# alshai/Big-BWT

Measured on AMD Instinct MI355X. Metric: input MB/s to .bwt (bit-exact vs ref), higher is better.
Workload: dtype u8; 1 GPU; BASELINE configs[2]: 64x mutated yeast-shaped FASTA (~0.79 GB), -w 10 -p 100, BWT + -s -e sampled SA; bytes_per_gpu=787308470, w=10, p=100, flags=6, phrases=16409159, words=921010, dict_bytes=79900101, parallelism=1 GPU

## Files before the change

### big-bwt_amd/csrc/merge.hip

```cpp
#include "kernels.hpp"
#include "prims.hpp"
#include "devutil.hpp"
#include <algorithm>
#include <cstdlib>

namespace pfp {

static constexpr int TB = 256;
constexpr int kOffTileLog = 11;


template <class I> struct alignas(16) Idx8 { I v[8]; };
template <class I>
__global__ __launch_bounds__(256) void slot_payload_kernel(uint64_t N, const I *__restrict__ sa,
                                                           const uint64_t *__restrict__ skeys,
                                                           const uint8_t *__restrict__ refined, const uint8_t *__restrict__ b,
                                                           WordView wv,
                                                           const uint32_t *__restrict__ wocc, uint32_t d, int w,
                                                           uint32_t *__restrict__ cnt, uint8_t *__restrict__ pc) {
  if ((uint64_t)BID * 2048 >= N) return;
  uint64_t t0 = ((uint64_t)BID * 256 + threadIdx.x) * 8;
  uint32_t c8[8], p8[8];
  const int nk = t0 >= N ? 0 : ((N - t0) >= 8 ? 8 : (int)(N - t0));
  uint64_t rf = 0;
// ... 110 lines not shown
  for (int q = 0; q < wv; q++) run += ws[q];
  uint32_t o8[8];
#pragma unroll
  for (int k = 0; k < 8; k++) { o8[k] = (uint32_t)run; run += r8[k].x; }
  *reinterpret_cast<uint4 *>(loc + t0) = make_uint4(o8[0], o8[1], o8[2], o8[3]);
  *reinterpret_cast<uint4 *>(loc + t0 + 4) = make_uint4(o8[4], o8[5], o8[6], o8[7]);
  if (threadIdx.x == 255) {
    tsum[BID] = run;
    if (run >> 32) atomicOr(overflow, 1u);
  }
  if (nk == 8) {
    *reinterpret_cast<uint2 *>(pc + t0) = make_uint2(p8[0] | (p8[1] << 8) | (p8[2] << 16) | (p8[3] << 24),
                                                     p8[4] | (p8[5] << 8) | (p8[6] << 16) | (p8[7] << 24));
    if (sfirst) {
      *reinterpret_cast<uint4 *>(sfirst + t0) = make_uint4(r8[0].y, r8[1].y, r8[2].y, r8[3].y);
      *reinterpret_cast<uint4 *>(sfirst + t0 + 4) = make_uint4(r8[4].y, r8[5].y, r8[6].y, r8[7].y);
    }
    if (slast) {
      *reinterpret_cast<uint4 *>(slast + t0) = make_uint4(r8[0].z, r8[1].z, r8[2].z, r8[3].z);
      *reinterpret_cast<uint4 *>(slast + t0 + 4) = make_uint4(r8[4].z, r8[5].z, r8[6].z, r8[7].z);
    }
    if (ssl) {
      *reinterpret_cast<uint4 *>(ssl + t0) = make_uint4(r8[0].w >> 8, r8[1].w >> 8, r8[2].w >> 8, r8[3].w >> 8);
      *reinterpret_cast<uint4 *>(ssl + t0 + 4) = make_uint4(r8[4].w >> 8, r8[5].w >> 8, r8[6].w >> 8, r8[7].w >> 8);
    }
  } else {
    for (int k = 0; k < nk; k++) {
      pc[t0 + k] = (uint8_t)p8[k];
      if (sfirst) sfirst[t0 + k] = r8[k].y;
      if (slast) slast[t0 + k] = r8[k].z;
      if (ssl) ssl[t0 + k] = r8[k].w >> 8;
    }
  }
#pragma unroll
  for (int k = 0; k < 8; k++) {
    if (k < nk && p8[k] != 0 && g8[k] == prev_g && (any_multi_is_hard || p8[k] != prev_pc)) hard[g8[k]] = 1;
    prev_pc = p8[k]; prev_g = g8[k];
  }
}

template <class I>
__global__ void group_flags_kernel(uint64_t N, const I *__restrict__ grp, const uint8_t *__restrict__ pc,
                                   int any_multi_is_hard, uint8_t *__restrict__ hard) {
  uint64_t t = (uint64_t)BID * blockDim.x + threadIdx.x;
  if (t >= N || pc[t] == 0) return;
  I g = grp[t];
  if (g == t) return;
  if (any_multi_is_hard || pc[t] != pc[g]) hard[g] = 1;
}

enum : uint8_t { CLS_NONE = 0, CLS_FILL = 1, CLS_FULL = 2, CLS_HARD = 3 };
enum : int { SA_NONE = 0, SA_DENSE = 1, SA_SPARSE = 2 };

template <class I>
__global__ void gather_idx_kernel(uint64_t n, const I *__restrict__ idx, const I *__restrict__ src, I *__restrict__ dst) {
  uint64_t i = (uint64_t)BID * blockDim.x + threadIdx.x;
  if (i < n) dst[i] = src[idx[i]];
}
struct alignas(32) WordRec { uint32_t ist, occ, first, last; uint64_t wend, pad; };
__global__ void wistart_kernel(uint32_t d, const uint32_t *__restrict__ lexrank, const uint32_t *__restrict__ istart_lex,
                               const uint32_t *__restrict__ wocc, const uint32_t *__restrict__ ilist,
                               const uint64_t *__restrict__ wend, uint32_t *__restrict__ wistart, WordRec *__restrict__ wrec) {
  uint32_t j = BID * blockDim.x + threadIdx.x;
  if (j >= d) return;
  const uint32_t st = istart_lex[lexrank[j]] + 1;
  wistart[j] = st;
  if (wrec) { const uint32_t oc = wocc[j]; wrec[j] = WordRec{st, oc, ilist[st], ilist[st + oc - 1], wend[j], 0}; }
}

template <class I>
struct MergeArgsT {
  uint64_t N, n_out; uint32_t d; int w; int want_sa;
  uint64_t pos_base, n_out_global;
  uint64_t out_lo, out_hi;
  const I *sa, *grp;
  WordView wv;
  const uint32_t *ist, *wistart;
  const WordRec *wrec;
  const uint32_t *sfirst, *slast, *ssl;
  const uint8_t *pc, *hard, *gmaj;
  const uint64_t *tbase; const uint32_t *loc;
  const uint32_t *ilist; const uint8_t *bwlast; const uint64_t *bwsai;
  const uint32_t *istart_lex, *iword; const uint64_t *wslot_lex; uint64_t slot_base;
  uint8_t *bwt; uint64_t *out_sa;
  int pass;
  const uint64_t *bmap, *bpre;
  uint64_t *sa_c;
};
enum : int { PASS_BWT = 1, PASS_SA = 2 };
template <class I>
__device__ __forceinline__ void sa_put(const MergeArgsT<I> &a, uint64_t x, uint64_t v) {
  if (x < a.out_lo || x >= a.out_hi) return;
  if (!a.bmap) { a.out_sa[x] = v; return; }
  const uint64_t r = x - a.out_lo, wv = a.bmap[r >> 6];
  if (!((wv >> (r & 63)) & 1ull)) return;
  if (a.sa_c) a.sa_c[a.bpre[r >> 6] + (uint64_t)__popcll(wv & ((1ull << (r & 63)) - 1ull))] = v;
  else a.out_sa[x] = v;
}
template <class I>
__device__ __forceinline__ bool sa_wanted(const MergeArgsT<I> &a, uint64_t x) {
  if (x < a.out_lo || x >= a.out_hi) return false;
  if (!a.bmap) return true;
  const uint64_t r = x - a.out_lo;
  return (a.bmap[r >> 6] >> (r & 63)) & 1ull;
}
template <class I>
__device__ __forceinline__ uint64_t slot_off(const MergeArgsT<I> &a, uint64_t t) { return a.tbase[t >> kOffTileLog] + a.loc[t]; }


__device__ __forceinline__ uint8_t fix_char(uint8_t ch) { return ch == kDollar ? 0 : ch; }
template <class I>
__device__ __forceinline__ uint32_t slot_ist(const MergeArgsT<I> &a, uint64_t t) {
  return a.ist ? a.ist[t] : a.wistart[word_of(a.wv, a.sa[t])];
}

template <class I>
__device__ __forceinline__ uint32_t slot_first(const MergeArgsT<I> &a, uint64_t t) { return a.sfirst ? a.sfirst[t] : a.wrec[word_of(a.wv, a.sa[t])].first; }
template <class I>
__device__ __forceinline__ uint32_t slot_last(const MergeArgsT<I> &a, uint64_t t) { return a.slast ? a.slast[t] : a.wrec[word_of(a.wv, a.sa[t])].last; }
template <class I>
__device__ __forceinline__ uint64_t slot_slen(const MergeArgsT<I> &a, uint64_t t) {
  if (a.ssl) { const uint32_t v = a.ssl[t]; if (v != kSlCap) return v; }
  return slen_of(a.wv, a.sa[t]);
}

constexpr int kHardLds = 1024;
constexpr int kHardRank = 512;
constexpr int kHardMem = 256;
constexpr int kHardSortMin = 512;
constexpr int kSlots = 2048;
constexpr uint64_t kExpandQuota = 1u << 16;

template <bool kDense>
struct ExpandLds {
  uint32_t loff[kSlots + 1];
  uint8_t lch[kSlots];
  uint8_t lcls[kDense ? kSlots : 1];
  uint32_t lfist[kDense ? kSlots : 1];
};

template <class I, bool kDense>
__device__ __forceinline__ void expand_stage(const MergeArgsT<I> &a, ExpandLds<kDense> &L, uint64_t t0, int ns, uint64_t base) {
  for (int s = threadIdx.x; s <= ns; s += 256) L.loff[s] = (uint32_t)(slot_off(a, t0 + s) - base);
  for (int s = threadIdx.x; s < ns; s += 256) {
    const uint64_t t = t0 + s;
    const uint8_t pc = a.pc[t];
    uint8_t cls = pc == 0 ? CLS_NONE : (pc == kEndOfWord ? CLS_FULL : CLS_FILL);
    uint8_t ch = 0;
    if (cls == CLS_FILL) {
      ch = fix_char(pc);
      const I g = a.grp[t];
      if (a.hard[g]) {
// ... 83 lines not shown
    for (uint64_t x0 = kExpandQuota + ((uint64_t)BID * 256 + threadIdx.x) * 16; x0 < Ltot; x0 += (uint64_t)GDIM * 256 * 16)
      expand_16(a, L, ns, base, x0, Ltot);
    if constexpr (kDense)
      for (uint64_t x = kExpandQuota + (uint64_t)BID * 256 + threadIdx.x; x < Ltot; x += (uint64_t)GDIM * 256)
        expand_sa_1(a, L, t0, ns, base, x);
  }
}

template <class I>
__device__ __forceinline__ bool word_entry(const MergeArgsT<I> &a, uint64_t e, uint64_t &t, uint64_t &x) {
  const uint32_t q = a.iword[e + 1] - 1u;
  const uint64_t gs = a.wslot_lex[q];
  if (gs < a.slot_base || gs - a.slot_base >= a.N) return false;
  t = gs - a.slot_base;
  x = slot_off(a, t) + (e - (uint64_t)a.istart_lex[q]);
  return true;
}
template <class I>
__global__ __launch_bounds__(256) void word_chars_kernel(MergeArgsT<I> a, uint64_t P) {
  const uint64_t e = (uint64_t)BID * 256 + threadIdx.x;
  if (e >= P) return;
  uint64_t t, x;
  if (!word_entry(a, e, t, x) || x < a.out_lo || x >= a.out_hi) return;
  a.bwt[x] = a.bwlast[a.ilist[e + 1]];
}
template <class I>
__global__ __launch_bounds__(256) void word_sa_kernel(MergeArgsT<I> a, uint64_t P) {
  const uint64_t e = (uint64_t)BID * 256 + threadIdx.x;
  if (e >= P) return;
  uint64_t t, x;
  if (!word_entry(a, e, t, x) || !sa_wanted(a, x)) return;
  const uint64_t pos = a.ilist[e + 1];
  sa_put(a, x, a.pos_base + x == 0 ? a.n_out_global - 1 : a.bwsai[pos] - slot_slen(a, t));
}
__global__ void iword_kernel(uint64_t P, uint32_t d, const uint32_t *__restrict__ istart_lex, uint32_t *__restrict__ iword) {
  const uint64_t e = (uint64_t)BID * blockDim.x + threadIdx.x;
  if (e > P) return;
  if (e == P) { iword[0] = 0; return; }
  uint32_t lo = 0, hi = d;
  while (hi - lo > 1) { const uint32_t mid = (lo + hi) >> 1; if ((uint64_t)istart_lex[mid] <= e) lo = mid; else hi = mid; }
  iword[e + 1] = lo + 1;
}

__device__ __forceinline__ uint32_t lane_read(uint32_t v, int l) { return (uint32_t)__builtin_amdgcn_readlane((int)v, l); }
__device__ __forceinline__ uint64_t lane_read(uint64_t v, int l) {
  return (uint64_t)lane_read((uint32_t)v, l) | ((uint64_t)lane_read((uint32_t)(v >> 32), l) << 32);
}
template <class I>
__global__ __launch_bounds__(256) void unit_edges_kernel(MergeArgsT<I> a) {
  const uint64_t t = (uint64_t)BID * 256 + threadIdx.x;
  const int lane = threadIdx.x & 63;
  const uint64_t wbase = t - lane;
  const bool in = t < a.N;
  const uint32_t ch = in ? a.pc[t] : 0u;
  const bool unit = ch != 0 && ch != kEndOfWord;
  I g = 0;
  if (unit) g = a.grp[t];
  const unsigned long long um = __ballot(unit);
  const I g_next = __shfl_down(g, 1, 64);
  const bool unit_next = (um >> ((lane + 1) & 63)) & 1ull;
  bool cont;
  if (lane < 63) cont = unit && unit_next && g_next == g;
  else cont = unit && t + 1 < a.N && a.pc[t + 1] != 0 && a.pc[t + 1] != kEndOfWord && a.grp[t + 1] == g;
  const unsigned long long cm = __ballot(cont);
  const bool head = unit && (uint64_t)g == t;
  const bool last = unit && !cont;
  uint64_t o_first = 0, o_last = 0;
  if (head) o_first = slot_off(a, t);
  if (last) o_last = slot_off(a, t + 1) - 1;
  const bool need_first = head && sa_wanted(a, o_first);
  const bool need_last = last && sa_wanted(a, o_last);
  const bool head_here = unit && (uint64_t)g >= wbase;
  const int hl = head_here ? (int)((uint64_t)g - wbase) : lane;
  const unsigned long long lm = __ballot(last) >> lane;
  const int ll = lm ? lane + (__ffsll((long long)lm) - 1) : lane;
  const bool nf = head_here && ((__ballot(need_first) >> hl) & 1ull);
  const bool nlz = unit && lm != 0 && ((__ballot(need_last) >> ll) & 1ull);
  uint32_t mn = 0xFFFFFFFFu, mx = 0;
  uint64_t mysl = 0;
  if (nf || nlz) {
    if (nf) mn = slot_first(a, t);
    if (nlz) mx = slot_last(a, t);
    if (need_first || need_last) mysl = slot_slen(a, t);
  }
  const bool do_min = __ballot(nf) != 0, do_max = __ballot(nlz) != 0;
  unsigned long long r = cm & ~(1ull << 63);
#pragma unroll
  for (int o = 1; o < 64; o <<= 1) {
    if (!r) break;
    if (do_min) {
      const uint32_t v = __shfl_down(mn, o, 64);
      if (((r >> lane) & 1ull) && v < mn) mn = v;
    }
    if (do_max) {
      const uint32_t v = __shfl_up(mx, o, 64);
      if (lane >= o && ((r >> (lane - o)) & 1ull) && v > mx) mx = v;
    }
    r &= r >> o;
  }
  const I g63 = lane_read(g, 63);
  const bool cont63 = (cm >> 63) & 1ull;
  const unsigned long long fwd = __ballot(need_first && cont63 && g63 == g);
  if (fwd) {
    uint32_t ext = 0xFFFFFFFFu;
    for (uint64_t m0 = wbase + 64;; m0 += 64) {
      const uint64_t m = m0 + lane;
      const bool mine = m < a.N && a.grp[m] == g63;
      uint32_t f = 0xFFFFFFFFu;
      if (mine) f = slot_first(a, m);
      f = wave_min(f);
      ext = f < ext ? f : ext;
      if (__ballot(mine) != ~0ull) break;
    }
    if ((fwd >> lane) & 1ull) mn = ext < mn ? ext : mn;
  }
  const uint64_t g0 = lane_read(g, 0);
  const unsigned long long bwd = __ballot(need_last && (uint64_t)g < wbase);
  if (bwd && (um & 1ull)) {
    uint32_t ext = 0;
    for (uint64_t m0 = g0; m0 < wbase; m0 += 64) {
      const uint64_t m = m0 + lane;
      uint32_t l = 0;
      if (m < wbase) l = slot_last(a, m);
      l = wave_max(l);
      ext = l > ext ? l : ext;
    }
    if ((bwd >> lane) & 1ull) mx = ext > mx ? ext : mx;
  }
  if (need_first) sa_put(a, o_first, a.bwsai[mn] - mysl);
  if (need_last) sa_put(a, o_last, a.bwsai[mx] - mysl);
}

__device__ __forceinline__ uint32_t pack_byte_flags(uint32_t m) {
  return (m & 1u) | ((m >> 7) & 2u) | ((m >> 14) & 4u) | ((m >> 21) & 8u);
}
__global__ __launch_bounds__(256) void run_bitmap_kernel(const uint8_t *__restrict__ bwt, uint64_t cnt, uint64_t *__restrict__ bmap,
                                                         uint32_t *__restrict__ wcnt, uint64_t *__restrict__ smap,
                                                         uint32_t *__restrict__ scnt, uint64_t *__restrict__ emap,
                                                         uint32_t *__restrict__ ecnt) {
  const uint64_t ch = (uint64_t)BID * 256 + threadIdx.x;
  const uint64_t base = ch * 16;
  uint32_t ms[4], me[4];
  run_mask16(bwt, base, cnt, -1, -1, 0, ms);
  run_mask16(bwt, base, cnt, -1, -1, 1, me);
  uint32_t bs = 0, be = 0;
#pragma unroll
  for (int q = 0; q < 4; q++) { bs |= pack_byte_flags(ms[q]) << (4 * q); be |= pack_byte_flags(me[q]) << (4 * q); }
  uint64_t vs = (uint64_t)bs << (16 * (threadIdx.x & 3)), ve = (uint64_t)be << (16 * (threadIdx.x & 3));
  vs |= __shfl_xor(vs, 1, 64); vs |= __shfl_xor(vs, 2, 64);
  ve |= __shfl_xor(ve, 1, 64); ve |= __shfl_xor(ve, 2, 64);
  if ((threadIdx.x & 3) == 0 && base < cnt) {
    const uint64_t w = ch >> 2;
    bmap[w] = vs | ve; wcnt[w] = (uint32_t)__popcll(vs | ve);
    if (smap) { smap[w] = vs; scnt[w] = (uint32_t)__popcll(vs); }
    if (emap) { emap[w] = ve; ecnt[w] = (uint32_t)__popcll(ve); }
  }
}
__global__ void count_unset_kernel(const uint64_t *__restrict__ v, uint64_t n, unsigned long long *__restrict__ total) {
  const uint64_t i = (uint64_t)BID * blockDim.x + threadIdx.x;
  if (i < n && v[i] == ~0ull) atomicAdd(total, 1ull);
}
struct HardGroupInfo { uint64_t g; uint64_t E; uint32_t k; uint32_t minor; };
struct MinorMember { uint64_t g; uint32_t k, m; uint64_t roff; uint64_t base; uint32_t ist, occ; uint32_t sl; uint32_t ch; };
struct MinorRec { uint64_t o; uint32_t pos, pred, succ, flags, sl, pad; };
template <class I>
__global__ __launch_bounds__(256) void hard_classify_kernel(MergeArgsT<I> a, const I *__restrict__ heads, uint64_t nH,
                                                            uint8_t *__restrict__ gmaj, HardGroupInfo *__restrict__ info,
                                                            uint32_t *__restrict__ minor_cnt, uint8_t *__restrict__ fallback,
                                                            unsigned long long *__restrict__ chars_total, uint32_t *__restrict__ minor_members) {
  const uint64_t h = (uint64_t)BID * 256 + threadIdx.x;
  unsigned long long mychars = 0, myk = 0;
  if (h < nH) {
  const uint64_t g = heads[h];
  uint64_t lo = 1, hi = 2;
  while (g + hi < a.N && a.grp[g + hi] == (I)g) { lo = hi; hi *= 2; }
  if (g + hi > a.N) hi = a.N - g;
  while (hi - lo > 1) { const uint64_t mid = (lo + hi) >> 1; if (a.grp[g + mid] == (I)g) lo = mid; else hi = mid; }
  const uint64_t k = hi;
  const uint64_t base = slot_off(a, g);
  const uint64_t E = slot_off(a, g + k) - base;
  uint32_t c0 = 0x100, c1 = 0x100, c2 = 0x100, c3 = 0x100;
  uint64_t n0 = 0, n1 = 0, n2 = 0, n3 = 0;
  bool many = false;
// ... 99 lines not shown
          bool hp = false, hs = false;
          if (m == me) {
            lb = j;
            if (a.want_sa) {
              if (j > 0) { pv = a.ilist[my_ist + j - 1]; hp = true; }
              if (j + 1 < my_occ) { sv = a.ilist[my_ist + j + 1]; hs = true; }
            }
          } else {
            const uint32_t mfirst = slot_first(a, g + m), mlast = slot_last(a, g + m);
            if (pos < mfirst) { lb = 0; sv = mfirst; hs = true; }
            else if (pos > mlast) { lb = (uint32_t)(slot_off(a, g + m + 1) - slot_off(a, g + m)); pv = mlast; hp = true; }
            else {
              const WordRec wr = a.wrec[word_of(a.wv, a.sa[g + m])];
              const uint32_t *lst = a.ilist + wr.ist;
              uint32_t l2 = 1, h2 = wr.occ - 1;
              while (l2 < h2) { const uint32_t mid = (l2 + h2) >> 1; if (lst[mid] < pos) l2 = mid + 1; else h2 = mid; }
              lb = l2;
              if (a.want_sa) { pv = lst[lb - 1]; hp = true; sv = lst[lb]; hs = true; }
            }
          }
          r += lb;
          if (hp && (!has_pred || pv > pred)) { pred = pv; has_pred = 1; }
          if (hs && (!has_succ || sv < succ)) { succ = sv; has_succ = 1; }
        }
      }
#pragma unroll
      for (int o = 1; o < LPM; o <<= 1) {
        r += __shfl_xor(r, o, 64);
        const uint32_t op = __shfl_xor(pred, o, 64), ohp = __shfl_xor(has_pred, o, 64);
        const uint32_t os = __shfl_xor(succ, o, 64), ohs = __shfl_xor(has_succ, o, 64);
        if (ohp && (!has_pred || op > pred)) { pred = op; has_pred = 1; }
        if (ohs && (!has_succ || os < succ)) { succ = os; has_succ = 1; }
      }
      if (!act || ll != 0) continue;
      const uint64_t o = base + r;
      if (o >= a.out_lo && o < a.out_hi) a.bwt[o] = mych;
      if (a.want_sa)
        recs[mmv.roff + j] = MinorRec{o, pos, pred, succ, has_pred | (has_succ << 1), (uint32_t)sl, 0u};
    }
  }
}

template <class I>
__global__ void hard_minor_sa_kernel(MergeArgsT<I> a, const MinorRec *__restrict__ recs, uint64_t n) {
  const uint64_t q = (uint64_t)BID * blockDim.x + threadIdx.x;
  if (q >= n) return;
  const MinorRec r = recs[q];
  sa_put(a, r.o, a.bwsai[r.pos] - (uint64_t)r.sl);
  if ((r.flags & 1u) && r.o >= 1) sa_put(a, r.o - 1, a.bwsai[r.pred] - (uint64_t)r.sl);
  if (r.flags & 2u) sa_put(a, r.o + 1, a.bwsai[r.succ] - (uint64_t)r.sl);
}

struct BigGroup { uint64_t g; uint64_t E; uint32_t k; uint32_t pad; };
struct HardLds {
  uint32_t lpos[kHardRank];
  uint8_t lq[kHardRank];
  uint32_t lmoff[kHardMem + 1], lmist[kHardMem], lmsl[kHardMem];
  uint8_t lmch[kHardMem], lmg[kHardMem];
  uint64_t gbase[64], ghead[64];
  uint32_t geoff[65], gk0[65];
};
__device__ __forceinline__ void wave_lds_sync() {
  __builtin_amdgcn_wave_barrier();
  __threadfence_block();
}
__device__ __forceinline__ uint32_t wave_max_u32(uint32_t v) {
#pragma unroll
  for (int o = 32; o > 0; o >>= 1) { const uint32_t x = __shfl_xor(v, o, 64); v = x > v ? x : v; }
  return v;
}
template <class I>
__global__ __launch_bounds__(256) void hard_groups_kernel(MergeArgsT<I> a, const I *__restrict__ heads,
                                                          const uint64_t *__restrict__ nheads_p,
                                                          unsigned long long *__restrict__ stats,
                                                          BigGroup *__restrict__ big, uint32_t big_cap,
                                                          BigGroup *__restrict__ mid, uint32_t mid_cap, int gpb) {
  __shared__ HardLds S[4];
  const int wv = threadIdx.x >> 6, lane = threadIdx.x & 63;
  HardLds &L = S[wv];
  const uint64_t nH = *nheads_p;
  const uint64_t nbatch = (nH + gpb - 1) / gpb;
  unsigned long long my_chars = 0, my_groups = 0;
  for (uint64_t b = BID * 4 + wv; b < nbatch; b += GDIM * 4) {
    const uint64_t hidx = b * gpb + lane;
    uint64_t g = 0, base = 0;
    uint32_t k = 0, E = 0;
    bool live = false;
    if (lane < gpb && hidx < nH) {
      g = heads[hidx];
      uint32_t kk = 0;
      while (g + kk < a.N && a.grp[g + kk] == (I)g && a.pc[g + kk] != 0) kk++;
      base = slot_off(a, g);
      const uint64_t Eg = slot_off(a, g + kk) - base;
      if (kk && !(base + Eg <= a.out_lo || base >= a.out_hi)) {
        my_chars += Eg; my_groups += 1;
        const bool sorted_path = Eg > (uint64_t)kHardSortMin;
        if (Eg <= (uint64_t)kHardRank && kk <= (uint32_t)kHardMem && !sorted_path) { live = true; k = kk; E = (uint32_t)Eg; }
        else if (Eg <= (uint64_t)kHardLds && sorted_path) {
          const unsigned long long idx = atomicAdd(&stats[3], 1ull);
          if (idx < mid_cap) mid[idx] = BigGroup{g, Eg, kk, 0};
        } else {
          const unsigned long long idx = atomicAdd(&stats[2], 1ull);
          if (idx < big_cap) big[idx] = BigGroup{g, Eg, kk, 0};
        }
      }
    }
    unsigned long long todo = __ballot(live);
    while (todo) {
      const bool mine = (todo >> lane) & 1ull;
      uint32_t pk = mine ? k : 0u, pE = mine ? E : 0u;
#pragma unroll
      for (int o = 1; o < 64; o <<= 1) {
        const uint32_t vk = __shfl_up(pk, o, 64), vE = __shfl_up(pE, o, 64);
        if (lane >= o) { pk += vk; pE += vE; }
      }
      const bool fit = mine && pk <= (uint32_t)kHardMem && pE <= (uint32_t)kHardRank;
      const unsigned long long take = __ballot(fit);
      todo &= ~take;
      const int nG = __popcll(take);
      const int lastl = 63 - __clzll((long long)take);
      const uint32_t M = __shfl(pk, lastl, 64), Eb = __shfl(pE, lastl, 64);
      if (fit) {
        const int gi = __popcll(take & ((1ull << lane) - 1ull));
        L.ghead[gi] = g; L.gbase[gi] = base; L.geoff[gi] = pE - E; L.gk0[gi] = pk - k;
      }
      if (lane == 0) { L.geoff[nG] = Eb; L.gk0[nG] = M; }
      wave_lds_sync();
      for (uint32_t q = lane; q < M; q += 64) {
        int lo = 0, hi = nG;
        while (hi - lo > 1) { const int mid = (lo + hi) >> 1; if (L.gk0[mid] <= q) lo = mid; else hi = mid; }
        const uint64_t t = L.ghead[lo] + (q - L.gk0[lo]);
        L.lmoff[q] = L.geoff[lo] + (uint32_t)(slot_off(a, t) - L.gbase[lo]);
        L.lmist[q] = slot_ist(a, t);
        uint32_t sl = 0;
        if (a.want_sa) sl = (uint32_t)slot_slen(a, t);
        L.lmsl[q] = sl;
        L.lmch[q] = fix_char(a.pc[t]);
        L.lmg[q] = (uint8_t)lo;
      }
      if (lane == 0) L.lmoff[M] = Eb;
      wave_lds_sync();
      for (uint32_t e = lane; e < Eb; e += 64) {
        uint32_t lo = 0, hi = M;
        while (hi - lo > 1) { const uint32_t mid = (lo + hi) >> 1; if (L.lmoff[mid] <= e) lo = mid; else hi = mid; }
        L.lpos[e] = a.ilist[L.lmist[lo] + (e - L.lmoff[lo])];
        L.lq[e] = (uint8_t)lo;
// ... 156 lines not shown
  }
  uint64_t own = 0;
  for (int k = 0; k < 8; k++) own += v[k];
  uint64_t inc = own;
  const int lane = threadIdx.x & 63, wv = threadIdx.x >> 6;
  for (int o = 1; o < 64; o <<= 1) { const uint64_t u = __shfl_up(inc, o, 64); if (lane >= o) inc += u; }
  if (lane == 63) ws[wv] = inc;
  __syncthreads();
  uint64_t run = inc - own;
  for (int q = 0; q < wv; q++) run += ws[q];
  uint32_t o8[8];
  for (int k = 0; k < 8; k++) { o8[k] = (uint32_t)run; run += v[k]; }
  *reinterpret_cast<uint4 *>(loc + t0) = make_uint4(o8[0], o8[1], o8[2], o8[3]);
  *reinterpret_cast<uint4 *>(loc + t0 + 4) = make_uint4(o8[4], o8[5], o8[6], o8[7]);
  if (threadIdx.x == 255) {
    tsum[BID] = run;
    if (run >> 32) atomicOr(overflow, 1u);
  }
}


enum class RecordSource {
  SortKeys,
  Gathered,
  PerSlot,
};

struct MergeSwitches {
  int prec_direct = -1;
  uint32_t big_cap = 0;
  uint64_t big_budget = 1ull << 27;
  static MergeSwitches read() {
    MergeSwitches s;
    if (const char *e = getenv("PFP_PREC_DIRECT")) s.prec_direct = atoi(e) != 0;
    if (const char *e = getenv("PFP_BIG_CAP")) { if (atoll(e) > 0) s.big_cap = (uint32_t)atoll(e); }
    if (const char *e = getenv("PFP_BIG_BUDGET")) s.big_budget = strtoull(e, nullptr, 10);
    return s;
  }
};

template <class I>
static RecordSource choose_record_source(pfp_ctx *c, uint64_t N, uint64_t NP, int sa_mode, const SuffixOrderT<I> &so, const MergeSwitches &sw) {
  if (sa_mode != SA_DENSE && so.paybits == 16 && so.skeys.p && so.n_refined * 5 < N) return RecordSource::SortKeys;
  bool direct = N * 4 <= NP;
  const uint64_t dev_bytes = c->pool.soft_limit ? c->pool.soft_limit / 7 * 10 : (64ull << 30);
  if (NP * sizeof(PosRec) > dev_bytes / 8) direct = true;
  if (sw.prec_direct >= 0) direct = sw.prec_direct != 0;
  return direct ? RecordSource::PerSlot : RecordSource::Gathered;
}

template <class I>
struct HeadList {
  const I *heads;
  const uint64_t *n_dev;
  uint64_t n;
};

template <class I>
struct Merge {
  pfp_ctx *const c;
  const Dictionary &D;
  const DictIndex &ix;
  const SuffixOrderT<I> &so;
  const ParseBWT &pb;
  const uint32_t *const occ_lex;
  const MergeOpts o;
  BwtOutputs &out;
  const uint64_t NP, N;
  const uint32_t d;
  const int sa_mode;
  const MergeSwitches sw;
  const RecordSource src;
  const WordView wv;
  const uint64_t ntile;
  const uint32_t nblk;
  const int first_pass;

  MergeArgsT<I> a{};
  uint64_t n_out = 0;

  struct {
    DBuf<uint32_t> istart_lex, wistart;
    DBuf<uint32_t> iword;
    DBuf<WordRec> wrec;
  } word;
  struct {
    DBuf<uint8_t> pc, hard;
    DBuf<uint32_t> loc, ovf;
    DBuf<uint64_t> tsum, tbase;
    DBuf<uint32_t> sfirst, slast, ssl;
  } slot;
  enum { kAllHeads = 0, kFallbackHeads = 1 };
  struct {
    DBuf<unsigned long long> hstats;
    uint64_t n_heads = 0;
    uint32_t big_cap = 0, mid_cap = 0;
    DBuf<BigGroup> big, mid;
    DBuf<I> heads;
    DBuf<uint64_t> list_len;
    DBuf<unsigned long long> mstat;
    DBuf<uint8_t> gmaj, fallback;
    DBuf<HardGroupInfo> ginfo;
    DBuf<uint32_t> minor_cnt, mm_cnt;
    DBuf<uint64_t> minor_off, mm_off;
    DBuf<MinorMember> mm_list;
    uint64_t n_mm = 0, sum_k = 0, n_minor = 0;
    DBuf<I> fb_heads;
    DBuf<MinorRec> recs;
    int gpb = 64;
    uint32_t nmid = 0, nbig = 0;
    DBuf<uint64_t> estart;
    std::vector<uint64_t> es;
  } hg;
  DBuf<uint32_t> heavy, nheavy;

  Merge(pfp_ctx *c_, const Dictionary &D_, const DictIndex &ix_, const SuffixOrderT<I> &so_, const ParseBWT &pb_, const uint32_t *occ_lex_,
        const MergeOpts &o_, BwtOutputs &out_)
      : c(c_), D(D_), ix(ix_), so(so_), pb(pb_), occ_lex(occ_lex_), o(o_), out(out_), NP(D_.dsize), N(so_.N), d((uint32_t)D_.d),
        sa_mode(!o_.flags ? SA_NONE : ((o_.flags & PFP_FLAG_SA) ? SA_DENSE : SA_SPARSE)), sw(MergeSwitches::read()),
        src(choose_record_source<I>(c_, N, NP, sa_mode, so_, sw)), wv(word_view(D_, ix_)), ntile((N >> kOffTileLog) + 1),
        nblk((uint32_t)cdiv64(N, kSlots)), first_pass(sa_mode == SA_SPARSE ? PASS_BWT : (PASS_BWT | PASS_SA)) {}

  MergeArgsT<I> with_pass(int pass) const { MergeArgsT<I> x = a; x.pass = pass; return x; }

  void word_records() {
    word.istart_lex.alloc(c, d); word.wistart.alloc(c, d);
    exclusive_sum_u32(c, occ_lex, word.istart_lex.p, d);
    word.wrec.alloc(c, d);
    hipLaunchKernelGGL(wistart_kernel, gdim(cdiv(d, TB)), gdim(TB), 0, c->stream, d, ix.lexrank.p, word.istart_lex.p, D.wocc.p, pb.ilist.p,
                       ix.wend.p, word.wistart.p, word.wrec.p);
    if (!pb.iword.p) {
      word.iword.alloc(c, pb.P + 1);
      hipLaunchKernelGGL(iword_kernel, gdim(cdiv(pb.P + 1, TB)), gdim(TB), 0, c->stream, pb.P, d, word.istart_lex.p, word.iword.p);
    }
  }

  void alloc_slot_tables() {
    slot.pc.alloc(c, N + 8); slot.hard.alloc(c, N);
    slot.loc.alloc(c, ntile << kOffTileLog); slot.ovf.alloc(c, 1);
    alloc_counts(c, slot.tsum, ntile); slot.tbase.alloc(c, ntile + 1);
    slot.hard.zero();
    slot.ovf.zero();
  }
  void slot_tables_from_keys(DBuf<uint32_t> &cnt) {
    { KScope ks(c, "pfp::slot_payload_kernel", N * (8 + 1 + 5));
      hipLaunchKernelGGL(slot_payload_kernel<I>, gdim(cdiv(cdiv64(N, 8), 256)), gdim(256), 0, c->stream, N, so.sa.p, so.skeys.p,
                         so.refined.p, D.bytes.p, wv, D.wocc.p, d, o.w, cnt.p, slot.pc.p); }
    { KScope ks(c, "pfp::slot_loc_kernel", N * 8);
      hipLaunchKernelGGL(slot_loc_kernel, gdim((unsigned)ntile), gdim(256), 0, c->stream, cnt.p, N, slot.loc.p, slot.tsum.p, slot.ovf.p); }
    { KScope ks(c, "pfp::group_flags_kernel", N * 5);
      hipLaunchKernelGGL(group_flags_kernel<I>, gdim(cdiv(N, TB)), gdim(TB), 0, c->stream, N, so.grp.p, slot.pc.p, 0, slot.hard.p); }
  }
  void slot_tables_gathered() {
    const int dense = sa_mode == SA_DENSE ? 1 : 0;
    const uint64_t np256 = cdiv64(NP, 256) * 256;
    DBuf<PosRec> prec(c, np256);
    { KScope ks(c, "pfp::pprec16_kernel", NP * (1 + 16) + (uint64_t)d * 40);
      hipLaunchKernelGGL(pprec16_kernel, gdim(cdiv(np256, TB)), gdim(TB), 0, c->stream, wv, o.w, reinterpret_cast<const uint4 *>(word.wrec.p),
                         dense, (uint64_t)0, NP, prec.p); }
    slot_records(prec.p);
// ... 21 lines not shown

  void fill_args() {
    const bool dense = sa_mode == SA_DENSE;
    a.N = N; a.n_out = n_out; a.d = d; a.w = o.w; a.want_sa = sa_mode;
    a.pos_base = o.pos_base; a.n_out_global = o.n_out_global ? o.n_out_global : n_out;
    a.sa = so.sa.p; a.grp = so.grp.p; a.wv = wv;
    a.ist = dense ? slot.sfirst.p : nullptr;
    a.wistart = word.wistart.p; a.wrec = word.wrec.p;
    a.sfirst = dense ? nullptr : slot.sfirst.p; a.slast = slot.slast.p; a.ssl = slot.ssl.p;
    a.pc = slot.pc.p; a.hard = slot.hard.p; a.tbase = slot.tbase.p; a.loc = slot.loc.p;
    a.ilist = pb.ilist.p; a.bwlast = pb.bwlast.p; a.bwsai = pb.bwsai.p;
    a.istart_lex = word.istart_lex.p; a.iword = pb.iword.p ? pb.iword.p : word.iword.p;
    a.wslot_lex = ix.wslot_lex.p; a.slot_base = so.slot_base;
    a.out_lo = o.out_lo; a.out_hi = o.out_hi < n_out ? o.out_hi : n_out;
    a.bwt = out.d_bwt - o.out_lo; a.out_sa = out.d_sa ? out.d_sa - o.out_lo : nullptr;
  }

  void find_hard_groups() {
    hg.hstats.alloc(c, 5);
    hg.hstats.zero();
    hg.n_heads = count_flags(c, slot.hard.p, N);
    hg.big_cap = sw.big_cap ? sw.big_cap : (uint32_t)std::min<uint64_t>({(uint64_t)1u << 20, hg.n_heads + 1, n_out / 1024 + 1});
    hg.big.alloc(c, hg.big_cap);
    hg.mid_cap = (uint32_t)std::min<uint64_t>(n_out / (kHardSortMin + 1) + 64, 0x7FFFFFFFull);
    hg.mid.alloc(c, hg.mid_cap);
    hg.heads.alloc(c, hg.n_heads + 1);
    hg.list_len.alloc(c, 2);
    select_index<I>(c, slot.hard.p, hg.heads.p, hg.list_len.p + kAllHeads, N);
    hg.mstat.alloc(c, 2);
    hg.mstat.zero();
  }

  HeadList<I> classify() {
    const uint64_t n_heads = hg.n_heads;
    hg.gmaj.alloc(c, N); hg.fallback.alloc(c, n_heads); hg.ginfo.alloc(c, n_heads);
    alloc_counts(c, hg.minor_cnt, n_heads); hg.minor_off.alloc(c, n_heads + 1);
    alloc_counts(c, hg.mm_cnt, n_heads); hg.mm_off.alloc(c, n_heads + 1);
    a.gmaj = hg.gmaj.p;
    { KScope ks(c, "pfp::hard_classify_kernel", n_heads * 40);
      hipLaunchKernelGGL(hard_classify_kernel<I>, gdim(cdiv(n_heads, 256)), gdim(256), 0, c->stream, a, hg.heads.p, n_heads, hg.gmaj.p,
                         hg.ginfo.p, hg.minor_cnt.p, hg.fallback.p, hg.mstat.p, hg.mm_cnt.p); }
    exclusive_sum_u32_u64(c, hg.minor_cnt.p, hg.minor_off.p, n_heads + 1);
    exclusive_sum_u32_u64(c, hg.mm_cnt.p, hg.mm_off.p, n_heads + 1);
    hg.n_mm = read_scalar(c, hg.mm_off.p + n_heads);
    hg.sum_k = read_scalar(c, (const uint64_t *)hg.mstat.p + 1);
    if (hg.n_mm) {
      hg.mm_list.alloc(c, hg.n_mm);
      KScope ks(c, "pfp::hard_minor_fill_kernel", n_heads * 40 + hg.n_mm * 16);
      hipLaunchKernelGGL(hard_minor_fill_kernel<I>, gdim(cdiv(n_heads * 8, 256)), gdim(256), 0, c->stream, a, hg.ginfo.p, n_heads, hg.mm_off.p,
                         hg.minor_off.p, hg.gmaj.p, hg.mm_list.p);
    }
    const uint64_t n_fallback = count_flags(c, hg.fallback.p, n_heads);
    hg.n_minor = read_scalar(c, hg.minor_off.p + n_heads);
    hg.fb_heads.alloc(c, n_fallback + 1);
    {
      DBuf<I> fidx(c, n_fallback + 1);
      select_index<I>(c, hg.fallback.p, fidx.p, hg.list_len.p + kFallbackHeads, n_heads);
      if (n_fallback) hipLaunchKernelGGL(gather_idx_kernel<I>, gdim(cdiv(n_fallback, 256)), gdim(256), 0, c->stream, n_fallback, fidx.p,
                                         hg.heads.p, hg.fb_heads.p);
      PFP_HIP(hipGetLastError());
      sync(c);
    }
    return HeadList<I>{hg.fb_heads.p, hg.list_len.p + kFallbackHeads, n_fallback};
  }

  void expand() {
    const MergeArgsT<I> ap = with_pass(first_pass);
    const bool dense = sa_mode == SA_DENSE;
    heavy.alloc(c, nblk); nheavy.alloc(c, 1);
    nheavy.zero();
    { KScope ks(c, "pfp::expand_kernel", N * (4 + 1 + sizeof(I) + 1) + n_out * (dense ? 17 : 1));
      if (dense) hipLaunchKernelGGL((expand_kernel<I, true>), gdim(nblk), gdim(256), 0, c->stream, ap, heavy.p, nheavy.p, nblk);
      else hipLaunchKernelGGL((expand_kernel<I, false>), gdim(nblk), gdim(256), 0, c->stream, ap, heavy.p, nheavy.p, nblk); }
    const uint32_t nh = read_scalar(c, nheavy.p);
    { KScope ks2(c, "pfp::expand_heavy_kernel", 0);
      if (nh && dense) hipLaunchKernelGGL((expand_heavy_kernel<I, true>), gdim(c->n_cu * 4), gdim(256), 0, c->stream, ap, heavy.p, nh);
      else if (nh) hipLaunchKernelGGL((expand_heavy_kernel<I, false>), gdim(c->n_cu * 4), gdim(256), 0, c->stream, ap, heavy.p, nh); }
    if (pb.P) {
      KScope ks(c, "pfp::word_chars_kernel", pb.P * (4 + 4 + 1 + 1) + (uint64_t)d * (8 + 4 + 12));
      hipLaunchKernelGGL(word_chars_kernel<I>, gdim(cdiv(pb.P, 256)), gdim(256), 0, c->stream, ap, pb.P);
    }
    PFP_HIP(hipGetLastError());
  }

  void place_minority(const HeadList<I> &lds) {
    if (hg.n_mm) {
      const MergeArgsT<I> ap = with_pass(first_pass);
      if (sa_mode == SA_SPARSE) hg.recs.alloc(c, hg.n_minor + 1);
      KScope ks(c, "pfp::hard_minor_kernel", hg.n_minor * 64);
      const uint64_t avg_k = hg.sum_k / std::max<uint64_t>(hg.n_heads - lds.n, 1);
      if (avg_k > 32)
        hipLaunchKernelGGL((hard_minor_kernel<I, 64>), gdim((unsigned)std::min<uint64_t>(cdiv64(hg.n_mm, 4), (uint64_t)c->n_cu * 64)), gdim(256), 0,
                           c->stream, ap, hg.mm_list.p, hg.n_mm, hg.recs.p);
      else
        hipLaunchKernelGGL((hard_minor_kernel<I, 8>), gdim((unsigned)std::min<uint64_t>(cdiv64(hg.n_mm, 32), (uint64_t)c->n_cu * 64)), gdim(256), 0,
                           c->stream, ap, hg.mm_list.p, hg.n_mm, hg.recs.p);
    }
    PFP_HIP(hipGetLastError());
  }

  void rank_in_lds(const HeadList<I> &lds) {
    const MergeArgsT<I> ap = with_pass(first_pass);
    while (hg.gpb > 8 && lds.n / hg.gpb < (uint64_t)c->n_cu * 32) hg.gpb >>= 1;
    for (;;) {
      if (!lds.n) { PFP_HIP(hipMemsetAsync(hg.hstats.p, 0, 40, c->stream)); }
      else { KScope ks(c, "pfp::hard_groups_kernel", N * 5);
        hipLaunchKernelGGL(hard_groups_kernel<I>, gdim(c->n_cu * 8), gdim(256), 0, c->stream, ap, lds.heads, lds.n_dev, hg.hstats.p, hg.big.p,
                           hg.big_cap, hg.mid.p, hg.mid_cap, hg.gpb); }
      PFP_HIP(hipGetLastError());
      PFP_HIP(hipMemcpyAsync(c->h_scalars, hg.hstats.p, 40, hipMemcpyDeviceToHost, c->stream));
      sync(c);
      if (c->h_scalars[2] <= hg.big_cap) break;
      hg.big_cap = (uint32_t)std::min<uint64_t>(c->h_scalars[2], 0xFFFFFFFFull);
      hg.big.alloc(c, hg.big_cap);
      hg.hstats.zero();
    }
    out.hard_chars = c->h_scalars[0];
    out.hard_groups = c->h_scalars[1];
    out.hard_minor_groups = hg.n_heads - lds.n; out.hard_minor_chars = hg.n_minor;
    out.hard_big_groups = c->h_scalars[2]; out.hard_max_members = c->h_scalars[4];
    hg.nmid = (uint32_t)std::min<uint64_t>(c->h_scalars[3], hg.mid_cap);
    PFP_REQUIRE(c->h_scalars[3] <= hg.mid_cap, PFP_EHIP, "more sorted-path hard groups than the output can hold");
    hg.nbig = (uint32_t)c->h_scalars[2];
    out.hard_chars += read_scalar(c, (const uint64_t *)hg.mstat.p);
    out.hard_groups += hg.n_heads - lds.n;
  }

  void lay_out_queued() {
    const uint32_t nbig = hg.nbig;
    hg.es.assign(nbig + 1, 0);
    if (!nbig) return;
    std::vector<BigGroup> hb(nbig);
    PFP_HIP(hipMemcpyAsync(hb.data(), hg.big.p, nbig * sizeof(BigGroup), hipMemcpyDeviceToHost, c->stream));
    sync(c);
    for (uint32_t q = 0; q < nbig; q++) hg.es[q + 1] = hg.es[q] + hb[q].E;
    hg.estart.alloc(c, nbig + 1);
    PFP_HIP(hipMemcpyAsync(hg.estart.p, hg.es.data(), (nbig + 1) * 8, hipMemcpyHostToDevice, c->stream));
    sync(c);
  }

  void queued_groups(int pass) {
    const MergeArgsT<I> ap = with_pass(pass);
    const std::vector<uint64_t> &es = hg.es;
    if (hg.nmid) {
      KScope ks(c, "pfp::hard_sort_kernel", (uint64_t)hg.nmid * (kHardSortMin + 1) * (sa_mode ? 21 : 5));
      hipLaunchKernelGGL(hard_sort_kernel<I>, gdim(c->n_cu * 4), gdim(256), 0, c->stream, ap, hg.mid.p, hg.nmid);
      PFP_HIP(hipGetLastError());
    }
    for (uint32_t q0 = 0; q0 < hg.nbig;) {
      uint32_t q1 = q0 + 1;
      while (q1 < hg.nbig && es[q1 + 1] - es[q0] <= sw.big_budget) q1++;
      const uint64_t cnt = es[q1] - es[q0];
      if (cnt > sw.big_budget) {
        const int nb = (int)std::min<uint64_t>(cdiv64(cnt, 256), (uint64_t)c->n_cu * 32);
        KScope ks(c, "pfp::hard_big_kernel", cnt * (sa_mode ? 21 : 5));
        hipLaunchKernelGGL(hard_big_kernel<I>, gdim(nb), gdim(256), 0, c->stream, ap, hg.big.p + q0, q1 - q0, hg.estart.p + q0, cnt);
      } else {
        DBuf<uint64_t> bk(c, cnt), bka(c, cnt), bv(c, cnt), bva(c, cnt);
        { KScope ks(c, "pfp::big_keys_kernel", cnt * 28);
          hipLaunchKernelGGL(big_keys_kernel<I>, gdim(cdiv(cnt, 256)), gdim(256), 0, c->stream, ap, hg.big.p, q0, q1, hg.estart.p, cnt, bk.p, bv.p); }
// ... 4 lines not shown
      PFP_HIP(hipGetLastError());
      q0 = q1;
    }
  }

  void mark_run_boundaries() {
    const uint64_t cnt_slice = a.out_hi > a.out_lo ? a.out_hi - a.out_lo : 0;
    const uint64_t nw = cdiv64(cnt_slice, 64);
    out.bmap.alloc(c, nw + 1); out.bpre.alloc(c, nw + 1);
    const bool want_s = !out.d_sa && (o.flags & PFP_FLAG_SSA), want_e = !out.d_sa && (o.flags & PFP_FLAG_ESA);
    out.slice_n = cnt_slice;
    {
      DBuf<uint32_t> wcnt, scnt, ecnt;
      alloc_counts(c, wcnt, nw);
      PFP_HIP(hipMemsetAsync(out.bmap.p + nw, 0, 8, c->stream));
      if (want_s) { out.smap.alloc(c, nw + 1); out.spre.alloc(c, nw + 1); alloc_counts(c, scnt, nw); }
      if (want_e) { out.emap.alloc(c, nw + 1); out.epre.alloc(c, nw + 1); alloc_counts(c, ecnt, nw); }
      if (nw) {
        KScope ks(c, "pfp::run_bitmap_kernel", cnt_slice + nw * (12 + (want_s ? 12 : 0) + (want_e ? 12 : 0)));
        hipLaunchKernelGGL(run_bitmap_kernel, gdim(cdiv(cdiv64(cnt_slice, 16), 256)), gdim(256), 0, c->stream, out.d_bwt, cnt_slice,
                           out.bmap.p, wcnt.p, out.smap.p, scnt.p, out.emap.p, ecnt.p);
      }
      exclusive_sum_u32_u64(c, wcnt.p, out.bpre.p, nw + 1);
      if (want_s) exclusive_sum_u32_u64(c, scnt.p, out.spre.p, nw + 1);
      if (want_e) exclusive_sum_u32_u64(c, ecnt.p, out.epre.p, nw + 1);
      out.n_bound = read_scalar(c, out.bpre.p + nw);
      if (want_s) out.n_starts = read_scalar(c, out.spre.p + nw);
      if (want_e) out.n_ends = read_scalar(c, out.epre.p + nw);
    }
    a.bmap = out.bmap.p; a.bpre = out.bpre.p;
    if (!out.d_sa) {
      out.sa_c.alloc(c, out.n_bound + 1);
      if (c->debug) PFP_HIP(hipMemsetAsync(out.sa_c.p, 0xFF, (out.n_bound + 1) * 8, c->stream));
      a.sa_c = out.sa_c.p;
    }
  }

  void sa_round(const HeadList<I> &lds) {
    const MergeArgsT<I> ap = with_pass(PASS_SA);
    if (pb.P) {
      KScope ks(c, "pfp::word_sa_kernel", pb.P * (4 + 1) + (uint64_t)d * (8 + 4 + 12) + out.n_bound * (4 + 8 + 8));
      hipLaunchKernelGGL(word_sa_kernel<I>, gdim(cdiv(pb.P, 256)), gdim(256), 0, c->stream, ap, pb.P);
    }
    { KScope ks(c, "pfp::unit_edges_kernel", N * (1 + sizeof(I) * 2 + 4));
      hipLaunchKernelGGL(unit_edges_kernel<I>, gdim(cdiv(N, 256)), gdim(256), 0, c->stream, ap); }
    if (hg.n_mm) {
      const uint64_t nr = hg.n_minor;
      if (nr) hipLaunchKernelGGL(hard_minor_sa_kernel<I>, gdim(cdiv(nr, 256)), gdim(256), 0, c->stream, ap, hg.recs.p, nr);
    }
    if (lds.n) {
      DBuf<unsigned long long> scratch(c, 5);
      scratch.zero();
      KScope ks(c, "pfp::hard_groups_kernel", N * 5);
      hipLaunchKernelGGL(hard_groups_kernel<I>, gdim(c->n_cu * 8), gdim(256), 0, c->stream, ap, lds.heads, lds.n_dev, scratch.p, hg.big.p,
                         0u, hg.mid.p, 0u, hg.gpb);
      PFP_HIP(hipGetLastError());
      queued_groups(PASS_SA);
      sync(c);
    }
    PFP_HIP(hipGetLastError());
  }

  void check_boundaries_set() {
    if (!c->debug || !a.sa_c) return;
    DBuf<unsigned long long> unset(c, 1);
    unset.zero();
    const uint64_t skip_lo = (a.pos_base + a.out_lo > 0) ? 1 : 0, skip_hi = (a.pos_base + a.out_hi < a.n_out_global) ? 1 : 0;
    if (out.n_bound > skip_lo + skip_hi)
      hipLaunchKernelGGL(count_unset_kernel, gdim(cdiv(out.n_bound, 256)), gdim(256), 0, c->stream, out.sa_c.p + skip_lo,
                         out.n_bound - skip_lo - skip_hi, unset.p);
    const uint64_t u = read_scalar(c, (const uint64_t *)unset.p);
    PFP_REQUIRE(u == 0, PFP_EHIP, "sparse SA: " + std::to_string(u) + " run boundaries of the BWT received no SA value");
  }

  void run() {
    PFP_REQUIRE(!o.flags || pb.bwsai.p, PFP_EINVAL, "SA output requested without sa info");
    PFP_REQUIRE(ix.wslot_lex.p, PFP_EINVAL, "merge: the dictionary index has no whole-word slots (compute_lexrank has not run)");
    word_records();
    {
      DBuf<uint32_t> cnt;
      if (src == RecordSource::SortKeys) alloc_counts(c, cnt, N, 8);
      alloc_slot_tables();
      switch (src) {
        case RecordSource::SortKeys: slot_tables_from_keys(cnt); break;
        case RecordSource::Gathered: slot_tables_gathered(); break;
        case RecordSource::PerSlot: slot_tables_per_slot(); break;
      }
      offsets_and_totals();
    }
    fill_args();
    find_hard_groups();
    const HeadList<I> lds = sa_mode != SA_DENSE && hg.n_heads ? classify() : HeadList<I>{hg.heads.p, hg.list_len.p + kAllHeads, hg.n_heads};
    expand();
    place_minority(lds);
    rank_in_lds(lds);
    lay_out_queued();
    queued_groups(first_pass);
    if (sa_mode == SA_SPARSE) {
      mark_run_boundaries();
      sa_round(lds);
      check_boundaries_set();
    }
    sync(c);
  }
};

template <class I>
void merge_bwt(pfp_ctx *c, const Dictionary &D, const DictIndex &ix, const SuffixOrderT<I> &so, const ParseBWT &pb,
               const uint32_t *occ_lex, const MergeOpts &o, BwtOutputs &out) {
  Merge<I>(c, D, ix, so, pb, occ_lex, o, out).run();
}
template void merge_bwt<uint32_t>(pfp_ctx *, const Dictionary &, const DictIndex &, const SuffixOrderT<uint32_t> &, const ParseBWT &,
                                  const uint32_t *, const MergeOpts &, BwtOutputs &);
template void merge_bwt<uint64_t>(pfp_ctx *, const Dictionary &, const DictIndex &, const SuffixOrderT<uint64_t> &, const ParseBWT &,
                                  const uint32_t *, const MergeOpts &, BwtOutputs &);

}
```

Baseline: 27090 MB/s.

## Precompute fallback group records and hoist unit_edges loads ahead of dependent logic

The hard-group kernel now receives precomputed fallback records (head, base offset, extent, member count) built once during classification, so it no longer walks each group's members and recomputes slot offsets on every pass. Separately, unit_edges_kernel issues its pc/grp/loc/tbase loads up front unconditionally and fetches the bitmap word and prefix once per edge, reusing them when writing the SA value. The aim is to cut serial dependent memory walks and duplicated bitmap lookups. In exchange it adds an extra record buffer, an extra kernel in classify, and loads that are now done even for non-unit slots, plus a debug-only consistency check.

```diff
diff --git a/big-bwt_amd/csrc/merge.hip b/big-bwt_amd/csrc/merge.hip
--- a/big-bwt_amd/csrc/merge.hip
+++ b/big-bwt_amd/csrc/merge.hip
@@ -186,11 +186,6 @@
 enum : uint8_t { CLS_NONE = 0, CLS_FILL = 1, CLS_FULL = 2, CLS_HARD = 3 };
 enum : int { SA_NONE = 0, SA_DENSE = 1, SA_SPARSE = 2 };
 
-template <class I>
-__global__ void gather_idx_kernel(uint64_t n, const I *__restrict__ idx, const I *__restrict__ src, I *__restrict__ dst) {
-  uint64_t i = (uint64_t)BID * blockDim.x + threadIdx.x;
-  if (i < n) dst[i] = src[idx[i]];
-}
 struct alignas(32) WordRec { uint32_t ist, occ, first, last; uint64_t wend, pad; };
 __global__ void wistart_kernel(uint32_t d, const uint32_t *__restrict__ lexrank, const uint32_t *__restrict__ istart_lex,
                                const uint32_t *__restrict__ wocc, const uint32_t *__restrict__ ilist,
@@ -232,6 +227,11 @@
   else a.out_sa[x] = v;
 }
 template <class I>
+__device__ __forceinline__ void sa_put_at(const MergeArgsT<I> &a, uint64_t x, uint64_t word, uint64_t pre, uint64_t v) {
+  if (a.bmap && a.sa_c) a.sa_c[pre + (uint64_t)__popcll(word & ((1ull << ((x - a.out_lo) & 63)) - 1ull))] = v;
+  else a.out_sa[x] = v;
+}
+template <class I>
 __device__ __forceinline__ bool sa_wanted(const MergeArgsT<I> &a, uint64_t x) {
   if (x < a.out_lo || x >= a.out_hi) return false;
   if (!a.bmap) return true;
@@ -421,24 +421,36 @@
   const int lane = threadIdx.x & 63;
   const uint64_t wbase = t - lane;
   const bool in = t < a.N;
-  const uint32_t ch = in ? a.pc[t] : 0u;
+  uint32_t ch = 0, ch_n = 0, loc_t = 0, loc_n = 0;
+  uint64_t tb_t = 0, tb_n = 0;
+  I g = 0, g_n = 0;
+  if (in) {
+    ch = a.pc[t]; g = a.grp[t];
+    loc_t = a.loc[t]; loc_n = a.loc[t + 1];
+    tb_t = a.tbase[t >> kOffTileLog]; tb_n = a.tbase[(t + 1) >> kOffTileLog];
+    if (lane == 63) { ch_n = a.pc[t + 1]; g_n = a.grp[t + 1]; }
+  }
   const bool unit = ch != 0 && ch != kEndOfWord;
-  I g = 0;
-  if (unit) g = a.grp[t];
+  if (!unit) g = 0;
   const unsigned long long um = __ballot(unit);
   const I g_next = __shfl_down(g, 1, 64);
   const bool unit_next = (um >> ((lane + 1) & 63)) & 1ull;
   bool cont;
   if (lane < 63) cont = unit && unit_next && g_next == g;
-  else cont = unit && t + 1 < a.N && a.pc[t + 1] != 0 && a.pc[t + 1] != kEndOfWord && a.grp[t + 1] == g;
+  else cont = unit && t + 1 < a.N && ch_n != 0 && ch_n != kEndOfWord && g_n == g;
   const unsigned long long cm = __ballot(cont);
   const bool head = unit && (uint64_t)g == t;
   const bool last = unit && !cont;
-  uint64_t o_first = 0, o_last = 0;
-  if (head) o_first = slot_off(a, t);
-  if (last) o_last = slot_off(a, t + 1) - 1;
-  const bool need_first = head && sa_wanted(a, o_first);
-  const bool need_last = last && sa_wanted(a, o_last);
+  const uint64_t o_first = tb_t + loc_t, o_last = tb_n + loc_n - 1;
+  const bool ask_first = head && o_first >= a.out_lo && o_first < a.out_hi;
+  const bool ask_last = last && o_last >= a.out_lo && o_last < a.out_hi;
+  uint64_t w_first = ~0ull, w_last = ~0ull, p_first = 0, p_last = 0;
+  if (a.bmap) {
+    if (ask_first) { const uint64_t k = (o_first - a.out_lo) >> 6; w_first = a.bmap[k]; p_first = a.bpre[k]; }
+    if (ask_last) { const uint64_t k = (o_last - a.out_lo) >> 6; w_last = a.bmap[k]; p_last = a.bpre[k]; }
+  }
+  const bool need_first = ask_first && ((w_first >> ((o_first - a.out_lo) & 63)) & 1ull);
+  const bool need_last = ask_last && ((w_last >> ((o_last - a.out_lo) & 63)) & 1ull);
   const bool head_here = unit && (uint64_t)g >= wbase;
   const int hl = head_here ? (int)((uint64_t)g - wbase) : lane;
   const unsigned long long lm = __ballot(last) >> lane;
@@ -496,8 +508,11 @@
     }
     if ((bwd >> lane) & 1ull) mx = ext > mx ? ext : mx;
   }
-  if (need_first) sa_put(a, o_first, a.bwsai[mn] - mysl);
-  if (need_last) sa_put(a, o_last, a.bwsai[mx] - mysl);
+  uint64_t v_first = 0, v_last = 0;
+  if (need_first) v_first = a.bwsai[mn];
+  if (need_last) v_last = a.bwsai[mx];
+  if (need_first) sa_put_at(a, o_first, w_first, p_first, v_first - mysl);
+  if (need_last) sa_put_at(a, o_last, w_last, p_last, v_last - mysl);
 }
 
 __device__ __forceinline__ uint32_t pack_byte_flags(uint32_t m) {
@@ -703,6 +718,26 @@
 }
 
 struct BigGroup { uint64_t g; uint64_t E; uint32_t k; uint32_t pad; };
+struct alignas(16) FallbackRec { uint64_t g, base, E; uint32_t k, pad; };
+template <class I>
+__global__ void fb_records_kernel(MergeArgsT<I> a, uint64_t n, const I *__restrict__ fidx, const HardGroupInfo *__restrict__ info,
+                                  I *__restrict__ fb_heads, FallbackRec *__restrict__ recs) {
+  const uint64_t i = (uint64_t)BID * blockDim.x + threadIdx.x;
+  if (i >= n) return;
+  const HardGroupInfo gi = info[fidx[i]];
+  fb_heads[i] = (I)gi.g;
+  recs[i] = FallbackRec{gi.g, slot_off(a, gi.g), gi.E, gi.k, 0u};
+}
+template <class I>
+__global__ void fb_records_check_kernel(MergeArgsT<I> a, uint64_t n, const FallbackRec *__restrict__ recs,
+                                        unsigned long long *__restrict__ bad) {
+  const uint64_t i = (uint64_t)BID * blockDim.x + threadIdx.x;
+  if (i >= n) return;
+  const FallbackRec r = recs[i];
+  uint64_t kk = 0;
+  while (r.g + kk < a.N && a.grp[r.g + kk] == (I)r.g && a.pc[r.g + kk] != 0) kk++;
+  if (kk != r.k || slot_off(a, r.g) != r.base || slot_off(a, r.g + kk) - r.base != r.E) atomicAdd(bad, 1ull);
+}
 struct HardLds {
   uint32_t lpos[kHardRank];
   uint8_t lq[kHardRank];
@@ -722,6 +757,7 @@
 }
 template <class I>
 __global__ __launch_bounds__(256) void hard_groups_kernel(MergeArgsT<I> a, const I *__restrict__ heads,
+                                                          const FallbackRec *__restrict__ recs ,
                                                           const uint64_t *__restrict__ nheads_p,
                                                           unsigned long long *__restrict__ stats,
                                                           BigGroup *__restrict__ big, uint32_t big_cap,
@@ -738,11 +774,17 @@
     uint32_t k = 0, E = 0;
     bool live = false;
     if (lane < gpb && hidx < nH) {
-      g = heads[hidx];
       uint32_t kk = 0;
-      while (g + kk < a.N && a.grp[g + kk] == (I)g && a.pc[g + kk] != 0) kk++;
-      base = slot_off(a, g);
-      const uint64_t Eg = slot_off(a, g + kk) - base;
+      uint64_t Eg;
+      if (recs) {
+        const FallbackRec r = recs[hidx];
+        g = r.g; kk = r.k; base = r.base; Eg = r.E;
+      } else {
+        g = heads[hidx];
+        while (g + kk < a.N && a.grp[g + kk] == (I)g && a.pc[g + kk] != 0) kk++;
+        base = slot_off(a, g);
+        Eg = slot_off(a, g + kk) - base;
+      }
       if (kk && !(base + Eg <= a.out_lo || base >= a.out_hi)) {
         my_chars += Eg; my_groups += 1;
         const bool sorted_path = Eg > (uint64_t)kHardSortMin;
@@ -1005,6 +1047,7 @@
 template <class I>
 struct HeadList {
   const I *heads;
+  const FallbackRec *recs;
   const uint64_t *n_dev;
   uint64_t n;
 };
@@ -1059,6 +1102,7 @@
     DBuf<MinorMember> mm_list;
     uint64_t n_mm = 0, sum_k = 0, n_minor = 0;
     DBuf<I> fb_heads;
+    DBuf<FallbackRec> fb_recs;
     DBuf<MinorRec> recs;
     int gpb = 64;
     uint32_t nmid = 0, nbig = 0;
@@ -1186,16 +1230,23 @@
     }
     const uint64_t n_fallback = count_flags(c, hg.fallback.p, n_heads);
     hg.n_minor = read_scalar(c, hg.minor_off.p + n_heads);
-    hg.fb_heads.alloc(c, n_fallback + 1);
+    hg.fb_heads.alloc(c, n_fallback + 1); hg.fb_recs.alloc(c, n_fallback + 1);
     {
       DBuf<I> fidx(c, n_fallback + 1);
       select_index<I>(c, hg.fallback.p, fidx.p, hg.list_len.p + kFallbackHeads, n_heads);
-      if (n_fallback) hipLaunchKernelGGL(gather_idx_kernel<I>, gdim(cdiv(n_fallback, 256)), gdim(256), 0, c->stream, n_fallback, fidx.p,
-                                         hg.heads.p, hg.fb_heads.p);
+      if (n_fallback) hipLaunchKernelGGL(fb_records_kernel<I>, gdim(cdiv(n_fallback, 256)), gdim(256), 0, c->stream, a, n_fallback, fidx.p,
+                                         hg.ginfo.p, hg.fb_heads.p, hg.fb_recs.p);
       PFP_HIP(hipGetLastError());
       sync(c);
     }
-    return HeadList<I>{hg.fb_heads.p, hg.list_len.p + kFallbackHeads, n_fallback};
+    if (c->debug && n_fallback) {
+      DBuf<unsigned long long> bad(c, 1);
+      bad.zero();
+      hipLaunchKernelGGL(fb_records_check_kernel<I>, gdim(cdiv(n_fallback, 256)), gdim(256), 0, c->stream, a, n_fallback, hg.fb_recs.p, bad.p);
+      const uint64_t nb = read_scalar(c, (const uint64_t *)bad.p);
+      PFP_REQUIRE(nb == 0, PFP_EHIP, "merge: " + std::to_string(nb) + " fallback records differ from the walk over their group's members");
+    }
+    return HeadList<I>{hg.fb_heads.p, hg.fb_recs.p, hg.list_len.p + kFallbackHeads, n_fallback};
   }
 
   void expand() {
@@ -1239,7 +1290,7 @@
     for (;;) {
       if (!lds.n) { PFP_HIP(hipMemsetAsync(hg.hstats.p, 0, 40, c->stream)); }
       else { KScope ks(c, "pfp::hard_groups_kernel", N * 5);
-        hipLaunchKernelGGL(hard_groups_kernel<I>, gdim(c->n_cu * 8), gdim(256), 0, c->stream, ap, lds.heads, lds.n_dev, hg.hstats.p, hg.big.p,
+        hipLaunchKernelGGL(hard_groups_kernel<I>, gdim(c->n_cu * 8), gdim(256), 0, c->stream, ap, lds.heads, lds.recs, lds.n_dev, hg.hstats.p, hg.big.p,
                            hg.big_cap, hg.mid.p, hg.mid_cap, hg.gpb); }
       PFP_HIP(hipGetLastError());
       PFP_HIP(hipMemcpyAsync(c->h_scalars, hg.hstats.p, 40, hipMemcpyDeviceToHost, c->stream));
@@ -1350,7 +1401,7 @@
       DBuf<unsigned long long> scratch(c, 5);
       scratch.zero();
       KScope ks(c, "pfp::hard_groups_kernel", N * 5);
-      hipLaunchKernelGGL(hard_groups_kernel<I>, gdim(c->n_cu * 8), gdim(256), 0, c->stream, ap, lds.heads, lds.n_dev, scratch.p, hg.big.p,
+      hipLaunchKernelGGL(hard_groups_kernel<I>, gdim(c->n_cu * 8), gdim(256), 0, c->stream, ap, lds.heads, lds.recs, lds.n_dev, scratch.p, hg.big.p,
                          0u, hg.mid.p, 0u, hg.gpb);
       PFP_HIP(hipGetLastError());
       queued_groups(PASS_SA);
@@ -1388,7 +1439,7 @@
     }
     fill_args();
     find_hard_groups();
-    const HeadList<I> lds = sa_mode != SA_DENSE && hg.n_heads ? classify() : HeadList<I>{hg.heads.p, hg.list_len.p + kAllHeads, hg.n_heads};
+    const HeadList<I> lds = sa_mode != SA_DENSE && hg.n_heads ? classify() : HeadList<I>{hg.heads.p, nullptr, hg.list_len.p + kAllHeads, hg.n_heads};
     expand();
     place_minority(lds);
     rank_in_lds(lds);
```

Measured after the change: 27450 MB/s, median of 6. +1.3%, better.
